# Daniel-Liu-c0deb0t/cute-nucleotides

Hardware: AMD Instinct MI355X
Metric: Gnt/s encode+decode on 16 GiB random ACGT; % HBM read roofline at 1/8 GPU (higher is better)
Workload: dtype u8

## Files before the change

hip/minimizer_kernels.hpp:

```cpp
#pragma once

#include <hip/hip_runtime.h>
#include <stdint.h>

#include "counted_output.hpp"
#include "kmer_kernels.hpp"
#include "util_kernels.hpp"

namespace cnt {

constexpr int kMinBlock = 256;
constexpr uint32_t kMinTile = 2048, kMinMaxW = 256;
constexpr uint32_t kMinEntries = kMinTile + kMinMaxW;
constexpr int kMinRounds = (int)(kMinEntries / kMinBlock);
constexpr int kMinWinRounds = (int)(kMinTile / kMinBlock);
constexpr int kMinWaves = kMinBlock / 64;
static_assert(kMinEntries % kMinBlock == 0 && kMinTile % kMinBlock == 0 && kMinEntries < 65536, "local indices are u16");

__device__ __forceinline__ uint64_t minimizer_kmer(const uint64_t* __restrict__ in, uint64_t last_word, uint64_t i, uint32_t k,
                                                   bool canonical) {
    const uint64_t wd = i >> 5;
    const uint32_t sh = 2u * ((uint32_t)i & 31u);
    const uint64_t lo = in[wd], hi = in[wd + 1 <= last_word ? wd + 1 : last_word];
    const uint64_t x = funnel64(lo, hi, sh) & (~0ull >> (64 - 2 * k));
    return canonical ? kmer_finish<true>(x, k) : kmer_finish<false>(x, k);
}

template <bool WRITE>
__global__ __launch_bounds__(kMinBlock) void minimizer_tiles(const uint64_t* __restrict__ in, uint64_t len, uint32_t k, uint32_t w,
                                                             uint32_t canonical, uint64_t first_tile, uint32_t* __restrict__ counts,
                                                             const uint64_t* __restrict__ offs, uint64_t* __restrict__ pos,
                                                             uint64_t* __restrict__ val, uint64_t out_cap) {
    __shared__ uint64_t s_h[kMinEntries];
    __shared__ uint16_t s_i[kMinEntries];
    __shared__ uint32_t s_cnt[kMinWinRounds * kMinWaves];
    __shared__ uint64_t s_base;
    const uint64_t tile = first_tile + blockIdx.x, t0 = tile * kMinTile;
    const uint64_t m = len - k + 1, n_win = m - w + 1, last_word = (len - 1) >> 5;
    const uint32_t lane = threadIdx.x, wave = lane >> 6, n_ent = kMinTile + w;
    const bool canon = canonical != 0;

    uint64_t ch[kMinRounds];
    uint16_t ci[kMinRounds];
#pragma unroll
    for (int r = 0; r < kMinRounds; ++r) {
        const uint32_t e = r * kMinBlock + lane;
        const uint64_t i = t0 + e - 1;
        ch[r] = e < n_ent && i < m ? fmix64(minimizer_kmer(in, last_word, i, k, canon)) : ~0ull;
        ci[r] = (uint16_t)e;
        if (e < n_ent) {
            s_h[e] = ch[r];
            s_i[e] = (uint16_t)e;
        }
    }
    __syncthreads();
    uint32_t d = 1;
    for (; 2 * d <= w; d <<= 1) {
        uint32_t changed = 0;
#pragma unroll
        for (int r = 0; r < kMinRounds; ++r) {
            const uint32_t e = r * kMinBlock + lane;
            if (e + d < n_ent) {
                const uint64_t hb = s_h[e + d];
                if (hb < ch[r]) {
                    ch[r] = hb;
                    ci[r] = s_i[e + d];
                    changed |= 1u << r;
                }
            }
        }
        __syncthreads();
#pragma unroll
        for (int r = 0; r < kMinRounds; ++r) {
            if (changed & (1u << r)) {
                const uint32_t e = r * kMinBlock + lane;
                s_h[e] = ch[r];
                s_i[e] = ci[r];
            }
        }
        __syncthreads();
    }
    const uint32_t off = w - d;
    auto argmin = [&](uint32_t s) -> uint32_t { return s_h[s + off] < s_h[s] ? s_i[s + off] : s_i[s]; };
    uint64_t ballots[kMinWinRounds];
    uint32_t p[kMinWinRounds];
#pragma unroll
    for (int r = 0; r < kMinWinRounds; ++r) {
        const uint32_t s = r * kMinBlock + lane + 1;
        const uint64_t t = t0 + s - 1;
        p[r] = argmin(s);
        const bool fresh = t < n_win && (t == 0 || p[r] != argmin(s - 1));
        ballots[r] = __ballot(fresh);
        if ((lane & 63) == 0) s_cnt[r * kMinWaves + wave] = (uint32_t)__popcll(ballots[r]);
    }
    __syncthreads();
    if (!WRITE) {
        if (lane == 0) {
            uint64_t c = 0;
            for (int q = 0; q < kMinWinRounds * kMinWaves; ++q) c += s_cnt[q];
            counts[tile] = (uint32_t)c;
        }
        return;
    }
    if (lane == 0) {
        uint32_t c = 0;
        for (int q = 0; q < kMinWinRounds * kMinWaves; ++q) {
            const uint32_t x = s_cnt[q];
            s_cnt[q] = c;
            c += x;
        }
        s_base = counted_tile_base(offs, counts, tile);
    }
    __syncthreads();
    const uint64_t base = s_base;
#pragma unroll
    for (int r = 0; r < kMinWinRounds; ++r) {
        const uint64_t b = ballots[r];
        if (!((b >> (lane & 63)) & 1)) continue;
        const uint32_t rank = __builtin_amdgcn_mbcnt_hi((uint32_t)(b >> 32), __builtin_amdgcn_mbcnt_lo((uint32_t)b, 0u));
        const uint64_t j = base + s_cnt[r * kMinWaves + wave] + rank;
        if (j >= out_cap) continue;
        const uint64_t i = t0 + p[r] - 1;
        __builtin_nontemporal_store(i, pos + j);
        if (val) __builtin_nontemporal_store(minimizer_kmer(in, last_word, i, k, canon), val + j);
    }
}

}
```

Baseline: 5483.

## Compute minimizer hashes with rolling k-mers per thread and compact outputs via LDS

Each thread now hashes a contiguous run of k-mers by rolling the forward and reverse-complement codes from three loaded words, instead of re-loading and re-extracting every k-mer. The doubling min-scan drops the changed-bitmask branches in favour of unconditional selects and writes. The neighbour argmin is obtained with a wave shuffle instead of a second LDS lookup. Output indices are compacted into shared memory so the position and value stores are written contiguously by consecutive lanes. The costs are strided LDS writes with possible bank conflicts, an extra barrier, and more unconditional LDS traffic in the scan.

```diff
diff --git a/hip/minimizer_kernels.hpp b/hip/minimizer_kernels.hpp
--- a/hip/minimizer_kernels.hpp
+++ b/hip/minimizer_kernels.hpp
@@ -16,6 +16,7 @@
 constexpr int kMinWinRounds = (int)(kMinTile / kMinBlock);
 constexpr int kMinWaves = kMinBlock / 64;
 static_assert(kMinEntries % kMinBlock == 0 && kMinTile % kMinBlock == 0 && kMinEntries < 65536, "local indices are u16");
+static_assert((kMinRounds - 1) * kMinBlock + kMinMaxW / 2 <= kMinEntries, "a doubling step of all rounds but the last stays inside the arrays");
 
 __device__ __forceinline__ uint64_t minimizer_kmer(const uint64_t* __restrict__ in, uint64_t last_word, uint64_t i, uint32_t k,
                                                    bool canonical) {
@@ -26,6 +27,32 @@
     return canonical ? kmer_finish<true>(x, k) : kmer_finish<false>(x, k);
 }
 
+template <bool CANONICAL>
+__device__ __forceinline__ void minimizer_block_hashes(const uint64_t* __restrict__ in, uint64_t last_word, uint64_t j1, uint32_t k,
+                                                       uint32_t valid, uint64_t* __restrict__ h) {
+    const int64_t wd = (int64_t)(j1 - 1) >> 5;
+    const uint32_t ph = (uint32_t)(j1 - 1) & 31u;
+    uint64_t wv[3];
+#pragma unroll
+    for (int j = 0; j < 3; ++j) {
+        const int64_t a = wd + j < 0 ? 0 : wd + j;
+        wv[j] = in[(uint64_t)a <= last_word ? (uint64_t)a : last_word];
+    }
+    const uint64_t mask = ~0ull >> (64 - 2 * k);
+    const uint32_t q = ph + k;
+    const uint32_t tail = (uint32_t)funnel64(q < 32 ? wv[0] : wv[1], q < 32 ? wv[1] : wv[2], 2u * (q & 31u));
+    uint64_t x = funnel64(wv[0], wv[1], 2u * ph) & mask, rc = 0;
+    if constexpr (CANONICAL) rc = reverse_codes64(x ^ 0xAAAAAAAAAAAAAAAAull) >> (64 - 2 * k);
+#pragma unroll
+    for (int r = 0; r < kMinRounds; ++r) {
+        const uint64_t v = CANONICAL && rc < x ? rc : x;
+        h[r] = (valid >> r) & 1u ? fmix64(v) : ~0ull;
+        const uint64_t code = (tail >> (2 * r)) & 3u;
+        x = (x >> 2) | (code << (2 * k - 2));
+        if constexpr (CANONICAL) rc = ((rc << 2) | (code ^ 2u)) & mask;
+    }
+}
+
 template <bool WRITE>
 __global__ __launch_bounds__(kMinBlock) void minimizer_tiles(const uint64_t* __restrict__ in, uint64_t len, uint32_t k, uint32_t w,
                                                              uint32_t canonical, uint64_t first_tile, uint32_t* __restrict__ counts,
@@ -33,7 +60,7 @@
                                                              uint64_t* __restrict__ val, uint64_t out_cap) {
     __shared__ uint64_t s_h[kMinEntries];
     __shared__ uint16_t s_i[kMinEntries];
-    __shared__ uint32_t s_cnt[kMinWinRounds * kMinWaves];
+    __shared__ uint32_t s_cnt[kMinWinRounds * kMinWaves + 1];
     __shared__ uint64_t s_base;
     const uint64_t tile = first_tile + blockIdx.x, t0 = tile * kMinTile;
     const uint64_t m = len - k + 1, n_win = m - w + 1, last_word = (len - 1) >> 5;
@@ -42,41 +69,48 @@
 
     uint64_t ch[kMinRounds];
     uint16_t ci[kMinRounds];
+    {
+        const uint32_t e0 = kMinRounds * lane;
+        const uint64_t j1 = t0 + e0;
+        uint64_t hi = e0 < n_ent ? n_ent - e0 : 0;
+        const uint64_t left = j1 <= m ? m + 1 - j1 : 0;
+        hi = hi < left ? hi : left;
+        const uint32_t valid = ((1u << (hi < (uint64_t)kMinRounds ? (uint32_t)hi : (uint32_t)kMinRounds)) - 1u) & ~(uint32_t)(j1 == 0);
+        if (canon)
+            minimizer_block_hashes<true>(in, last_word, j1, k, valid, ch);
+        else
+            minimizer_block_hashes<false>(in, last_word, j1, k, valid, ch);
 #pragma unroll
-    for (int r = 0; r < kMinRounds; ++r) {
-        const uint32_t e = r * kMinBlock + lane;
-        const uint64_t i = t0 + e - 1;
-        ch[r] = e < n_ent && i < m ? fmix64(minimizer_kmer(in, last_word, i, k, canon)) : ~0ull;
-        ci[r] = (uint16_t)e;
-        if (e < n_ent) {
-            s_h[e] = ch[r];
-            s_i[e] = (uint16_t)e;
+        for (int r = 0; r < kMinRounds; ++r) {
+            s_h[e0 + r] = ch[r];
+            s_i[r * kMinBlock + lane] = (uint16_t)(r * kMinBlock + lane);
         }
     }
     __syncthreads();
+#pragma unroll
+    for (int r = 0; r < kMinRounds; ++r) {
+        ch[r] = s_h[r * kMinBlock + lane];
+        ci[r] = (uint16_t)(r * kMinBlock + lane);
+    }
     uint32_t d = 1;
     for (; 2 * d <= w; d <<= 1) {
-        uint32_t changed = 0;
 #pragma unroll
         for (int r = 0; r < kMinRounds; ++r) {
             const uint32_t e = r * kMinBlock + lane;
-            if (e + d < n_ent) {
+            if (r < kMinRounds - 1 || e + d < kMinEntries) {
                 const uint64_t hb = s_h[e + d];
-                if (hb < ch[r]) {
-                    ch[r] = hb;
-                    ci[r] = s_i[e + d];
-                    changed |= 1u << r;
-                }
+                const uint16_t ib = s_i[e + d];
+                const bool take = hb < ch[r];
+                ch[r] = take ? hb : ch[r];
+                ci[r] = take ? ib : ci[r];
             }
         }
         __syncthreads();
 #pragma unroll
         for (int r = 0; r < kMinRounds; ++r) {
-            if (changed & (1u << r)) {
-                const uint32_t e = r * kMinBlock + lane;
-                s_h[e] = ch[r];
-                s_i[e] = ci[r];
-            }
+            const uint32_t e = r * kMinBlock + lane;
+            s_h[e] = ch[r];
+            s_i[e] = ci[r];
         }
         __syncthreads();
     }
@@ -89,7 +123,9 @@
         const uint32_t s = r * kMinBlock + lane + 1;
         const uint64_t t = t0 + s - 1;
         p[r] = argmin(s);
-        const bool fresh = t < n_win && (t == 0 || p[r] != argmin(s - 1));
+        uint32_t before = __shfl_up(p[r], 1, 64);
+        if ((lane & 63) == 0) before = argmin(s - 1);
+        const bool fresh = t < n_win && (t == 0 || p[r] != before);
         ballots[r] = __ballot(fresh);
         if ((lane & 63) == 0) s_cnt[r * kMinWaves + wave] = (uint32_t)__popcll(ballots[r]);
     }
@@ -109,18 +145,23 @@
             s_cnt[q] = c;
             c += x;
         }
+        s_cnt[kMinWinRounds * kMinWaves] = c;
         s_base = counted_tile_base(offs, counts, tile);
     }
     __syncthreads();
-    const uint64_t base = s_base;
 #pragma unroll
     for (int r = 0; r < kMinWinRounds; ++r) {
         const uint64_t b = ballots[r];
-        if (!((b >> (lane & 63)) & 1)) continue;
         const uint32_t rank = __builtin_amdgcn_mbcnt_hi((uint32_t)(b >> 32), __builtin_amdgcn_mbcnt_lo((uint32_t)b, 0u));
-        const uint64_t j = base + s_cnt[r * kMinWaves + wave] + rank;
-        if (j >= out_cap) continue;
-        const uint64_t i = t0 + p[r] - 1;
+        if ((b >> (lane & 63)) & 1) s_i[s_cnt[r * kMinWaves + wave] + rank] = (uint16_t)p[r];
+    }
+    __syncthreads();
+    const uint64_t base = s_base;
+    const uint32_t n_out = s_cnt[kMinWinRounds * kMinWaves];
+    for (uint32_t q = lane; q < n_out; q += kMinBlock) {
+        const uint64_t j = base + q;
+        if (j >= out_cap) break;
+        const uint64_t i = t0 + s_i[q] - 1;
         __builtin_nontemporal_store(i, pos + j);
         if (val) __builtin_nontemporal_store(minimizer_kmer(in, last_word, i, k, canon), val + j);
     }
```

After: 5481, median of 2. About the same (-0.0%).
